# shionhonda/gae-dgl

Measured on AMD Instinct MI355X. Metric: edges aggregated/sec (SpMM fwd+bwd), higher is better.
Workload: dtype f32 (storage, aggregations, accumulators; the dense products run on the 16-bit matrix pipe from split operands with fp32 accumulation: X W^T and dW from three bf16 pieces per operand / six pairs, the loss from two fp16 pieces (N >= 5120) or three bf16 pieces -- all fp32-grade, see ms_per_step_exact_

## Files before the change

### gae_dgl_amd/csrc/common.h

```cpp
#pragma once
#include <hip/hip_runtime.h>
#include <stdint.h>
#include <stdio.h>

#include <atomic>

#include "gae_hip.h"
#include "gae_hip_experimental.h"

namespace gae {

struct Knob {
    std::atomic<int> v;
    explicit constexpr Knob(int x) : v(x) {}
    operator int() const { return v.load(std::memory_order_relaxed); }
    Knob &operator=(int x) { v.store(x, std::memory_order_relaxed); return *this; }
};

extern Knob g_spmm_variant, g_spmm_rpg, g_spmm_tile_vecs, g_spmm_ell, g_spmm_ell_rpg, g_spmm_hot, g_spmm_desc, g_spmm_light;
extern Knob g_gemm_rows, g_linear_wlds, g_atb_bf16, g_ell_side;
extern Knob g_xw_rows, g_xw_parts, g_xw_glds, g_xw_p3;
extern Knob g_bce_s_bf16, g_bce_pv_bf16, g_bce_sym, g_bce_sym_ri, g_bce_sym_bal, g_bce_last_kind;
extern Knob g_topk_splits;

// ... 119 lines not shown
struct PartialList {
    const float *base;
    float *out;
    int64_t n, n_partials, stride, row_len, row_pitch, out_pitch;
};
int launch_partials_reduce(const PartialList &a, const PartialList &b, hipStream_t s);

__device__ __forceinline__ void philox_round(uint32_t (&c)[4], uint32_t k0, uint32_t k1)
{
    const uint64_t p0 = uint64_t(0xD2511F53u) * c[0];
    const uint64_t p1 = uint64_t(0xCD9E8D57u) * c[2];
    const uint32_t n0 = uint32_t(p1 >> 32) ^ c[1] ^ k0;
    const uint32_t n2 = uint32_t(p0 >> 32) ^ c[3] ^ k1;
    c[1] = uint32_t(p1); c[3] = uint32_t(p0); c[0] = n0; c[2] = n2;
}

__device__ __forceinline__ void philox4x32_10(uint64_t ctr, uint64_t draw, uint64_t seed, uint32_t (&c)[4])
{
    c[0] = uint32_t(ctr); c[1] = uint32_t(ctr >> 32); c[2] = uint32_t(draw); c[3] = uint32_t(draw >> 32);
    uint32_t k0 = uint32_t(seed), k1 = uint32_t(seed >> 32);
#pragma unroll
    for (int r = 0; r < 10; ++r) {
        philox_round(c, k0, k1);
        k0 += 0x9E3779B9u; k1 += 0xBB67AE85u;
    }
}

__device__ __forceinline__ float dropout_multiplier(uint32_t bits, float p, float scale)
{
    const float u = float(bits >> 8) * (1.0f / 16777216.0f);
    return u >= p ? scale : 0.f;
}

}
```

### gae_dgl_amd/csrc/decoder_bce.hip

```cpp
#include <string.h>

#include "common.h"
#include "bce_finalize.h"

namespace {

using gae::kWave;
typedef float f32x4 __attribute__((ext_vector_type(4)));
typedef short s16x4 __attribute__((ext_vector_type(4)));
typedef float f32x2 __attribute__((ext_vector_type(2)));
typedef __bf16 bf16x2 __attribute__((ext_vector_type(2)));

constexpr int TJ = 64;
constexpr int PREP_ROWS = 64;
constexpr int kBceRi = 2;
constexpr int64_t kBceGrid = 2048;
constexpr int64_t kBceSymGrid = 16384;
constexpr int kChipCus = 256;
}

namespace gae {
Knob g_bce_s_bf16{3};
Knob g_bce_last_kind{0};
Knob g_bce_sym_bal{1};
// ... 25 lines not shown
#pragma unroll
    for (int r = 0; r < 4; ++r) {
        t[r] = 1.0f + __builtin_amdgcn_exp2f(-fabsf(y[r]));
        tA += fabsf(y[r]);
    }
    float t01, t23, q;
    if constexpr (SCALAR_TREE) {
        asm("v_mul_f32 %0, %1, %2" : "=v"(t01) : "v"(t[0]), "v"(t[1]));
        asm("v_mul_f32 %0, %1, %2" : "=v"(t23) : "v"(t[2]), "v"(t[3]));
        asm("v_mul_f32 %0, %1, %2" : "=v"(q) : "v"(t01), "v"(t23));
    } else {
        t01 = t[0] * t[1]; t23 = t[2] * t[3]; q = t01 * t23;
    }
    tP *= q;
    const float R = __builtin_amdgcn_rcpf(q);
    const float r01 = R * t23, r23 = R * t01;
    float s0, s1, s2, s3;
    asm("v_fma_f32 %0, %1, %2, -0.5" : "=v"(s0) : "v"(r01), "v"(t[1]));
    asm("v_fma_f32 %0, %1, %2, -0.5" : "=v"(s1) : "v"(r01), "v"(t[0]));
    asm("v_fma_f32 %0, %1, %2, -0.5" : "=v"(s2) : "v"(r23), "v"(t[3]));
    asm("v_fma_f32 %0, %1, %2, -0.5" : "=v"(s3) : "v"(r23), "v"(t[2]));
    return f32x4{copysignf(s0, y[0]), copysignf(s1, y[1]), copysignf(s2, y[2]), copysignf(s3, y[3])};
}

__global__ __launch_bounds__(256) void bce_prepare_kernel(const float *__restrict__ Z, float *__restrict__ mask,
                                                          int64_t ldz, int64_t n, int d, int DP, int64_t row_begin,
                                                          int64_t row_end, float *__restrict__ Zt,
                                                          unsigned short *__restrict__ Zhi,
                                                          unsigned short *__restrict__ Zlo,
                                                          double *__restrict__ colsum_partial ,
                                                          float drop_p, float drop_scale, uint64_t seed,
                                                          uint64_t offset, const uint64_t *__restrict__ draw_dev,
                                                          const int64_t *__restrict__ counts ,
                                                          double *__restrict__ scal , double all_pairs)
{
    __shared__ double red[2][256];
    const int tid = threadIdx.x;
    const int64_t n_valid = counts ? counts[0] : n;
    if (counts && blockIdx.x == 0 && tid == 0) {
        const double nv = double(counts[0]), ev = double(counts[1]);
        scal[0] = ev > 0 ? (nv * nv - ev) / ev : 0.0;
        scal[1] = nv > 0 ? 1.0 / (nv * nv) : 0.0;
        scal[2] = all_pairs - nv * nv;
    }
    const int k = tid % DP, rl = tid / DP, rpp = 256 / DP;
    const int64_t r0 = int64_t(blockIdx.x) * PREP_ROWS;
    double s_all = 0.0, s_win = 0.0;
    const bool draw = drop_p > 0.f;
    const uint64_t draw_idx = (draw && draw_dev) ? *draw_dev : 0;
    for (int rr = rl; rr < PREP_ROWS; rr += rpp) {
        const int64_t i = r0 + rr;
        if (i >= n) break;
        float v = 0.f;
        if (k < d && i >= n_valid) {
            if (draw) mask[i * ldz + k] = 0.f;
        } else if (k < d) {
            v = Z[i * ldz + k];
            if (draw) {
                const int64_t e = i * d + k;
                uint32_t c[4];
                gae::philox4x32_10(offset + uint64_t(e >> 2), draw_idx, seed, c);
                const uint32_t bits = (e & 2) ? ((e & 1) ? c[3] : c[2]) : ((e & 1) ? c[1] : c[0]);
                const float m = gae::dropout_multiplier(bits, drop_p, drop_scale);
                mask[i * ldz + k] = m;
                v *= m;
            } else if (mask) {
                v *= mask[i * ldz + k];
            }
        }
        Zt[i * DP + k] = v;
        const unsigned short hi = gae::f32_to_bf16(v);
        Zhi[i * DP + k] = hi;
        Zlo[i * DP + k] = gae::f32_to_bf16(v - gae::bf16_to_f32(hi));
        s_all += double(v);
        if (i >= row_begin && i < row_end) s_win += double(v);
    }
    red[0][tid] = s_all; red[1][tid] = s_win;
    __syncthreads();
    if (tid < DP) {
        double a = 0.0, w = 0.0;
        for (int q = 0; q < rpp; ++q) { a += red[0][q * DP + tid]; w += red[1][q * DP + tid]; }
        colsum_partial[(int64_t(blockIdx.x) * 2 + 0) * DP + tid] = a;
        colsum_partial[(int64_t(blockIdx.x) * 2 + 1) * DP + tid] = w;
    }
}

__device__ __forceinline__ void bce_colsum_block(const double *__restrict__ colsum_partial, int64_t n_blocks, int DP,
                                                 double *__restrict__ S ,
                                                 float *__restrict__ S_all_f , double *red )
{
    const int k = threadIdx.x % DP, q = threadIdx.x / DP, nq = 256 / DP;
    double a = 0.0, w = 0.0;
    for (int64_t b = q; b < n_blocks; b += nq) {
        a += colsum_partial[(b * 2 + 0) * DP + k];
        w += colsum_partial[(b * 2 + 1) * DP + k];
    }
    red[threadIdx.x] = a; red[256 + threadIdx.x] = w;
    __syncthreads();
    if (threadIdx.x < DP) {
        a = 0.0; w = 0.0;
        for (int j = 0; j < nq; ++j) { a += red[j * DP + k]; w += red[256 + j * DP + k]; }
        S[k] = a; S[DP + k] = w;
        S_all_f[k] = float(a);
    }
}

typedef short s16x8 __attribute__((ext_vector_type(8)));
typedef __bf16 bf16x8 __attribute__((ext_vector_type(8)));
// ... 41 lines not shown
    unsigned h[2], l[2], l2[2];
#pragma unroll
    for (int q = 0; q < 2; ++q) {
        const f32x2 a = {v[2 * q], v[2 * q + 1]};
        const unsigned hu = __builtin_bit_cast(unsigned, __builtin_convertvector(a, bf16x2));
        const f32x2 r1 = a - f32x2{__uint_as_float(hu << 16), __uint_as_float(hu & 0xffff0000u)};
        const unsigned lu = __builtin_bit_cast(unsigned, __builtin_convertvector(r1, bf16x2));
        const f32x2 r2 = r1 - f32x2{__uint_as_float(lu << 16), __uint_as_float(lu & 0xffff0000u)};
        h[q] = hu; l[q] = lu;
        l2[q] = __builtin_bit_cast(unsigned, __builtin_convertvector(r2, bf16x2));
    }
    struct U { unsigned a, b; } uh{h[0], h[1]}, ul{l[0], l[1]}, ul2{l2[0], l2[1]};
    hi = __builtin_bit_cast(s16x4, uh);
    lo = __builtin_bit_cast(s16x4, ul);
    lo2 = __builtin_bit_cast(s16x4, ul2);
}
__device__ __forceinline__ s16x4 third_piece(const f32x4 &v, const s16x4 &hi, const s16x4 &lo)
{
    unsigned l2[2];
#pragma unroll
    for (int q = 0; q < 2; ++q) {
        const f32x2 a = {v[2 * q], v[2 * q + 1]};
        const f32x2 fh = {gae::bf16_to_f32((unsigned short)hi[2 * q]), gae::bf16_to_f32((unsigned short)hi[2 * q + 1])};
        const f32x2 fl = {gae::bf16_to_f32((unsigned short)lo[2 * q]), gae::bf16_to_f32((unsigned short)lo[2 * q + 1])};
        l2[q] = __builtin_bit_cast(unsigned, __builtin_convertvector((a - fh) - fl, bf16x2));
    }
    struct U { unsigned a, b; } u{l2[0], l2[1]};
    return __builtin_bit_cast(s16x4, u);
}

typedef _Float16 f16x8 __attribute__((ext_vector_type(8)));
typedef _Float16 f16x4 __attribute__((ext_vector_type(4)));
typedef __fp16 fp16x2 __attribute__((ext_vector_type(2)));
constexpr float kF16Max = 32768.f;
__device__ __forceinline__ f32x4 mfma32h(const s16x8 &a, const s16x8 &b, const f32x4 &c)
{
    return __builtin_amdgcn_mfma_f32_16x16x32_f16(__builtin_bit_cast(f16x8, a), __builtin_bit_cast(f16x8, b), c, 0, 0, 0);
}
template <bool F16>
__device__ __forceinline__ f32x4 mfma_k32(const s16x8 &a, const s16x8 &b, const f32x4 &c)
{
    if constexpr (F16) return mfma32h(a, b, c);
    else return mfma32(a, b, c);
}
typedef _Float16 f16x2 __attribute__((ext_vector_type(2)));
__device__ __forceinline__ float minus_f16_lo(float v, unsigned hh)
{
    float r;
    asm("v_fma_mix_f32 %0, %1, -1.0, %2 op_sel_hi:[1,0,0]" : "=v"(r) : "v"(hh), "v"(v));
    return r;
}
__device__ __forceinline__ float minus_f16_hi(float v, unsigned hh)
{
    float r;
    asm("v_fma_mix_f32 %0, %1, -1.0, %2 op_sel:[1,0,0] op_sel_hi:[1,0,0]" : "=v"(r) : "v"(hh), "v"(v));
    return r;
}
__device__ __forceinline__ void split_f16x4(const f32x4 &v, s16x4 &hi, s16x4 &lo)
{
    unsigned h[2], l[2];
#pragma unroll
    for (int q = 0; q < 2; ++q) {
        const f32x2 a = {v[2 * q], v[2 * q + 1]};
        const unsigned hu = __builtin_bit_cast(unsigned, __builtin_convertvector(a, f16x2));
        const f32x2 r = {minus_f16_lo(a[0], hu), minus_f16_hi(a[1], hu)};
        h[q] = hu;
        l[q] = __builtin_bit_cast(unsigned, __builtin_convertvector(r, f16x2));
// ... 285 lines not shown
    }
#pragma unroll
    for (int off = 32; off > 0; off >>= 1) { la += __shfl_down(la, off, 64); ll += __shfl_down(ll, off, 64); }
    if (lane == 0) { red[wave][0] = la; red[wave][1] = ll; }
    __syncthreads();
    if (tid == 0) {
        const int64_t b = int64_t(blockIdx.y) * n_row_blocks + blockIdx.x;
        loss_partial[2 * b + 0] = (red[0][0] + red[1][0]) + (red[2][0] + red[3][0]);
        loss_partial[2 * b + 1] = (red[0][1] + red[1][1]) + (red[2][1] + red[3][1]);
    }
}

}

namespace gae {
Knob g_bce_sym_ri{0};
}

namespace {
using gae::g_bce_sym_ri;

__device__ __forceinline__ s16x4 upper_halves(const f32x4 &d)
{
    struct U { unsigned a, b; } u{__builtin_amdgcn_perm(__float_as_uint(d[1]), __float_as_uint(d[0]), 0x07060302u),
                                  __builtin_amdgcn_perm(__float_as_uint(d[3]), __float_as_uint(d[2]), 0x07060302u)};
    return __builtin_bit_cast(s16x4, u);
}

__host__ __device__ inline int64_t sym_strip_offset(int64_t I, int64_t NP, int64_t PR)
{
    return 16 * (I * NP - PR * (I * (I + 1) / 2));
}

template <bool WITH_GRAD, int RI, bool TRV, bool S3 = false, bool F16 = false, bool PERSIST = false, bool BAL = false>
__global__ __launch_bounds__(256, (RI == 2 && !PERSIST) ? 3 : 2) void bce_dense_sym_kernel(
    const float *__restrict__ Zt , const unsigned short *__restrict__ Zhi,
    const unsigned short *__restrict__ Zlo, int64_t n, int64_t cols_per_chunk,
    float *__restrict__ O_partial , float *__restrict__ Wmir,
    double *__restrict__ loss_partial , const double *__restrict__ colsum_partial,
    int64_t n_prep_blocks, double *__restrict__ S, float *__restrict__ S_all_f, unsigned n_panels, int exp_strip,
    unsigned *__restrict__ range_flag, int flag_mode, unsigned ticket, unsigned n_chunks, int bal_tpb)
{
    if (flag_mode == 2 && *range_flag != ticket) return;
    static_assert(!(S3 && F16), "three bf16 pieces OR two fp16 pieces");
    bool out_of_range = false;
    constexpr bool STAGE32 = S3 || F16;
    constexpr int DP = 16, SYM_PR = 64 * RI;
    constexpr int LDH = DP + 4;
    constexpr int V4 = TJ * DP / 4 / 256;
    constexpr int LDT = TJ + 4;
    constexpr int LDM = TJ + 4;
    constexpr int LDHL = 2 * DP + 8;
    __shared__ __attribute__((aligned(16))) unsigned short HLs[2][TJ * LDHL];
    __shared__ __attribute__((aligned(16))) unsigned short L2s[2][S3 ? TJ * LDH : 4];
    __shared__ __attribute__((aligned(16))) unsigned short HT[2][TRV ? 4 : DP * LDT];
    __shared__ __attribute__((aligned(16))) unsigned short LT[2][TRV ? 4 : DP * LDT];
    __shared__ __attribute__((aligned(16))) float MR[2][4][16 * LDM];
    __shared__ double red[4][2];

  double sumA = 0.0, sumL = 0.0;
  auto unit = [&](const int64_t I, const int64_t col_begin, const int64_t col_end, const int64_t op_slot, const int64_t lp_index) {
    const int tid = threadIdx.x, lane = tid & 63, wave = tid >> 6;
    const int l15 = lane & 15, g = lane >> 4;
    const int64_t NP = (n + 63) / 64 * 64;
    const int64_t row_base = SYM_PR * I + wave * (RI * 16);
    const int64_t diag_end = SYM_PR * (I + 1);

    constexpr float LOG2E = 1.44269504088896341f;
    static_assert(RI % 2 == 0, "row subtiles are paired into K = 32 mirror products");
    s16x8 bhh[RI];
    s16x8 bll[RI];
    s16x8 b3[S3 ? RI : 1];
    s16x8 zTh[RI / 2], zTl[RI / 2];
#pragma unroll
    for (int ri = 0; ri < RI; ++ri) {
        const int64_t i = row_base + ri * 16 + l15;
        f32x4 b = *reinterpret_cast<const f32x4 *>(Zt + (i < n ? i : 0) * DP + 4 * g);
        if (i >= n) b = f32x4{0.f, 0.f, 0.f, 0.f};
        b *= LOG2E;
        s16x4 bhi, blo, blo2;
        if (S3) { split_bf16x4_3(b, bhi, blo, blo2); b3[ri] = cat(bhi, blo2); }
        else if (F16) {
            out_of_range |= !(fmaxf(fmaxf(fabsf(b[0]), fabsf(b[1])), fmaxf(fabsf(b[2]), fabsf(b[3]))) <= kF16Max * LOG2E);
            split_f16x4(b, bhi, blo);
        } else split_bf16x4(b, bhi, blo);
        bhh[ri] = cat(bhi, bhi);
        bll[ri] = cat(blo, blo);
        s16x4 th, tl;
#pragma unroll
        for (int r = 0; r < 4; ++r) {
            const int64_t ir = row_base + ri * 16 + 4 * g + r;
            const bool v = ir < n;
            if (F16) continue;
            th[r] = v ? short(Zhi[(v ? ir : 0) * DP + l15]) : short(0);
            tl[r] = v ? short(Zlo[(v ? ir : 0) * DP + l15]) : short(0);
        }
        if (F16) {
            f32x4 zr;
#pragma unroll
            for (int r = 0; r < 4; ++r) {
                const int64_t ir = row_base + ri * 16 + 4 * g + r;
                zr[r] = ir < n ? Zt[ir * DP + l15] : 0.f;
            }
            split_f16x4(zr, th, tl);
        }
        put_half(zTh[ri / 2], ri & 1, th);
        put_half(zTl[ri / 2], ri & 1, tl);
    }
    s16x4 ident;
#pragma unroll
    for (int r = 0; r < 4; ++r) ident[r] = (4 * g + r == l15) ? short(F16 ? 0x3C00 : 0x3F80) : short(0);
    f32x4 oacc[RI];
#pragma unroll
    for (int ri = 0; ri < RI; ++ri) oacc[ri] = f32x4{0.f, 0.f, 0.f, 0.f};
    if (!BAL) { sumA = 0.0; sumL = 0.0; }
    bool rvalid[RI];
#pragma unroll
    for (int ri = 0; ri < RI; ++ri) rvalid[ri] = (row_base + ri * 16 + l15) < n;
// ... 5 lines not shown
#pragma unroll
            for (int r = 0; r < 4; ++r) pad_lane += (pad_j0 + jt * 16 + 4 * g + r >= n) ? 1.f : 0.f;
    }

    struct Stage { s16x4 h[STAGE32 ? 1 : V4], l[STAGE32 ? 1 : V4]; f32x4 f[STAGE32 ? V4 : 1]; };
    auto load_tile = [&](int64_t j0, Stage &st) {
#pragma unroll
        for (int q = 0; q < V4; ++q) {
            const int idx = tid + 256 * q;
            const int jj = idx / (DP / 4), kk = (idx % (DP / 4)) * 4;
            const bool jv = j0 + jj < col_end;
            const int64_t j = jv ? j0 + jj : col_begin;
            if (STAGE32) {
                st.f[q] = *reinterpret_cast<const f32x4 *>(Zt + j * DP + kk);
                if (!jv) st.f[q] = f32x4{0.f, 0.f, 0.f, 0.f};
            } else {
                st.h[q] = *reinterpret_cast<const s16x4 *>(Zhi + j * DP + kk);
                st.l[q] = *reinterpret_cast<const s16x4 *>(Zlo + j * DP + kk);
                if (!jv) { st.h[q] = s16x4{0, 0, 0, 0}; st.l[q] = s16x4{0, 0, 0, 0}; }
            }
        }
    };
    auto store_tile = [&](int buf, const Stage &st) {
#pragma unroll
        for (int q = 0; q < V4; ++q) {
            const int idx = tid + 256 * q;
            const int jj = idx / (DP / 4), kk = (idx % (DP / 4)) * 4;
            s16x4 h4, l4;
            if (S3) {
                s16x4 l24;
                split_bf16x4_3(st.f[q], h4, l4, l24);
                *reinterpret_cast<s16x4 *>(&L2s[buf][jj * LDH + kk]) = l24;
            } else if (F16) {
                const f32x4 f = st.f[q];
                out_of_range |= !(fmaxf(fmaxf(fabsf(f[0]), fabsf(f[1])), fmaxf(fabsf(f[2]), fabsf(f[3]))) <= kF16Max);
                split_f16x4(f, h4, l4);
            } else {
                h4 = st.h[q]; l4 = st.l[q];
            }
            *reinterpret_cast<s16x8 *>(&HLs[buf][jj * LDHL + 2 * kk]) = cat(h4, l4);
            if (WITH_GRAD && !TRV) {
#pragma unroll
                for (int e = 0; e < 4; ++e) {
                    HT[buf][(kk + e) * LDT + jj] = (unsigned short)h4[e];
                    LT[buf][(kk + e) * LDT + jj] = (unsigned short)l4[e];
                }
            }
        }
    };
    float *strip = Wmir + sym_strip_offset(I, NP, SYM_PR);
    auto flush_mirror = [&](int64_t j0, int mb) {
        const int f = tid >> 4, jq = (tid & 15) * 4;
        f32x4 v = *reinterpret_cast<const f32x4 *>(&MR[mb][0][f * LDM + jq]);
#pragma unroll
        for (int w = 1; w < 4; ++w) v += *reinterpret_cast<const f32x4 *>(&MR[mb][w][f * LDM + jq]);
        f32x4 *sp = reinterpret_cast<f32x4 *>(strip + (j0 - diag_end) * 16 + f * TJ + jq);
        if (exp_strip == 1) __builtin_nontemporal_store(v, sp);
        else if (exp_strip == 2) asm volatile("global_store_dwordx4 %0, %1, off sc1" ::"v"(sp), "v"(v) : "memory");
        else *sp = v;
    };

    auto compute_tile = [&](int buf, int64_t j0, bool offdiag) {
        float tA[RI], tP[RI];
#pragma unroll
        for (int ri = 0; ri < RI; ++ri) { tA[ri] = 0.f; tP[ri] = 1.f; }
#pragma unroll((RI == 4 && S3) ? 1 : TJ / 32)
        for (int jp = 0; jp < TJ / 32; ++jp) {
            s16x8 ph[RI], pl[RI];
#pragma unroll
// ... 81 lines not shown
#pragma unroll
        for (int ri = 0; ri < RI; ++ri) {
            a += rvalid[ri] ? tA[ri] : 0.f;
            l += rvalid[ri] ? __builtin_amdgcn_logf(tP[ri]) - padcnt : 0.f;
        }
        sumA += w * double(a);
        sumL += w * double(l);
    };

    Stage stage;
    load_tile(col_begin, stage);
    store_tile(0, stage);
    __syncthreads();
    int buf = 0;
    for (int64_t j0 = col_begin; j0 < col_end; j0 += TJ, buf ^= 1) {
        const bool more = j0 + TJ < col_end;
        if (more) load_tile(j0 + TJ, stage);
        const bool offdiag = j0 >= diag_end;
        compute_tile(buf, j0, offdiag);
        if (more) store_tile(buf ^ 1, stage);
        __syncthreads();
        if (WITH_GRAD && offdiag) flush_mirror(j0, buf);
    }
    if (WITH_GRAD) {
        float *op = O_partial + op_slot * n * DP;
#pragma unroll
        for (int ri = 0; ri < RI; ++ri)
#pragma unroll
            for (int r = 0; r < 4; ++r) {
                const int64_t i = row_base + ri * 16 + 4 * g + r;
                if (i < n) op[i * DP + l15] = oacc[ri][r];
            }
    }
    if (F16 && flag_mode == 1 && out_of_range) atomicExch(range_flag, ticket);
    if (BAL) return;
    double la = sumA * 0.69314718055994531, ll = sumL;
#pragma unroll
    for (int off = 32; off > 0; off >>= 1) { la += __shfl_down(la, off, 64); ll += __shfl_down(ll, off, 64); }
    if (lane == 0) { red[wave][0] = la; red[wave][1] = ll; }
    __syncthreads();
    if (tid == 0) {
        loss_partial[2 * lp_index + 0] = (red[0][0] + red[1][0]) + (red[2][0] + red[3][0]);
        loss_partial[2 * lp_index + 1] = (red[0][1] + red[1][1]) + (red[2][1] + red[3][1]);
    }
  };
  auto unit_xy = [&](const unsigned bx, const unsigned by) {
    if (bx >= n_panels) {
        if (by == 0)
            bce_colsum_block(colsum_partial, n_prep_blocks, DP, S, S_all_f, reinterpret_cast<double *>(&MR[0][0][0]));
        return;
    }
    const int64_t col_begin = SYM_PR * int64_t(bx) + int64_t(by) * cols_per_chunk;
    const int64_t lp_index = int64_t(by) * n_panels + bx;
    if (col_begin >= n) {
        if (threadIdx.x == 0) { loss_partial[2 * lp_index] = 0.0; loss_partial[2 * lp_index + 1] = 0.0; }
        return;
    }
    const int64_t ce = col_begin + cols_per_chunk;
    unit(bx, col_begin, ce > n ? n : ce, by, lp_index);
  };
    if constexpr (BAL) {
        const unsigned n_vb = n_chunks;
        auto vblock = [&](const unsigned vb) {
        if (vb + 1 == n_vb) {
            bce_colsum_block(colsum_partial, n_prep_blocks, DP, S, S_all_f, reinterpret_cast<double *>(&MR[0][0][0]));
            return;
        }
// ... 6 lines not shown
        if (t1 > W) t1 = W;
        if (t0 < t1) {
            const float hb = float(NT) + 0.5f * float(TPP);
            int I = int((hb - sqrtf(fmaxf(hb * hb - 2.0f * float(TPP) * float(t0), 0.0f))) / float(TPP));
            if (I < 0) I = 0;
            if (I > T - 1) I = T - 1;
            I = __builtin_amdgcn_readfirstlane(I);
            while (I > 0 && prefix(I) > t0) --I;
            while (I + 1 < T && prefix(I + 1) <= t0) ++I;
            while (t0 < t1) {
                const int pI = prefix(I), tiles = NT - TPP * I;
                const int lt = t0 - pI;
                int cnt = tiles - lt;
                if (cnt > t1 - t0) cnt = t1 - t0;
                const int64_t cb = int64_t(SYM_PR) * I + int64_t(lt) * 64;
                int64_t ce = cb + int64_t(cnt) * 64;
                if (ce > n) ce = n;
                if (cb < n) unit(I, cb, ce, int(vb) - int(unsigned(pI) / unsigned(bal_tpb)), -1);
                __syncthreads();
                t0 += cnt; ++I;
            }
        }
        const int tid = threadIdx.x, lane = tid & 63, wave = tid >> 6;
        double la = sumA * 0.69314718055994531, ll = sumL;
#pragma unroll
        for (int off = 32; off > 0; off >>= 1) { la += __shfl_down(la, off, 64); ll += __shfl_down(ll, off, 64); }
        if (lane == 0) { red[wave][0] = la; red[wave][1] = ll; }
        __syncthreads();
        if (tid == 0) {
            loss_partial[2 * vb + 0] = (red[0][0] + red[1][0]) + (red[2][0] + red[3][0]);
            loss_partial[2 * vb + 1] = (red[0][1] + red[1][1]) + (red[2][1] + red[3][1]);
        }
        };
        if constexpr (PERSIST) {
            for (unsigned vb = blockIdx.x; vb < n_vb; vb += gridDim.x) {
                vblock(vb);
                __syncthreads();
            }
        } else {
            vblock(blockIdx.x);
        }
    } else if constexpr (PERSIST) {
        const unsigned nx = n_panels + 1, total = nx * n_chunks;
        for (unsigned u = blockIdx.x; u < total; u += gridDim.x) {
            unit_xy(u % nx, u / nx);
            __syncthreads();
        }
    } else {
        unit_xy(blockIdx.x, blockIdx.y);
    }
}

__global__ __launch_bounds__(256) void bce_mirror_reduce_kernel(const float *__restrict__ Wmir, int64_t n,
                                                               float *__restrict__ Omir , int SYM_PR)
{
    const int64_t NP = (n + 63) / 64 * 64;
    const int64_t j0 = int64_t(blockIdx.x) * TJ;
    const int f = threadIdx.x >> 4, jq = (threadIdx.x & 15) * 4;
    const int64_t n_left = j0 / SYM_PR;
    f32x4 acc = {0.f, 0.f, 0.f, 0.f};
    auto at = [&](int64_t I) {
        const int64_t de = SYM_PR * (I + 1);
        return *reinterpret_cast<const f32x4 *>(Wmir + sym_strip_offset(I, NP, SYM_PR) + (j0 - de) * 16 + f * TJ + jq);
    };
    int64_t I = 0;
    for (; I + 8 <= n_left; I += 8) {
        f32x4 v[8];
#pragma unroll
        for (int u = 0; u < 8; ++u) v[u] = at(I + u);
#pragma unroll
        for (int u = 0; u < 8; ++u) acc += v[u];
    }
    for (; I < n_left; ++I) acc += at(I);
#pragma unroll
    for (int e = 0; e < 4; ++e)
        if (j0 + jq + e < n) Omir[(j0 + jq + e) * 16 + f] = acc[e];
}

template <int VEC, int LPR, bool WITH_GRAD>
__global__ __launch_bounds__(256) void bce_edges_kernel(
    const float *__restrict__ Zt , const float *__restrict__ mask, int64_t ldz,
    int64_t row_begin, int64_t n_local, int d, const int32_t *__restrict__ indptr,
    const int32_t *__restrict__ indices, const int32_t *__restrict__ t_indptr, const int32_t *__restrict__ t_indices,
// ... 454 lines not shown
    GAE_REQUIRE((Z || prepared) && loss_out && workspace && (n_local == 0 || indptr), GAE_E_NULL, "gae_decoder_bce: NULL pointer");
    GAE_REQUIRE(!dZ || n_local == 0 || t_indptr, GAE_E_NULL, "gae_decoder_bce: the gradient needs the CSR of A^T");
    BcePlan p;
    bce_plan(n, n_local, d, true, p);
    GAE_REQUIRE(workspace_bytes >= p.total_bytes, GAE_E_WORKSPACE, "gae_decoder_bce: workspace %lld < %lld bytes",
                (long long)workspace_bytes, (long long)p.total_bytes);
    if (prepared) {
        GAE_REQUIRE(prepared_blocks >= 1 && prepared_blocks * 2 * p.DP * 8 <= p.cs_bytes, GAE_E_RANGE,
                    "gae_x_decoder_bce_prepared: %lld column-sum partials do not fit the workspace", (long long)prepared_blocks);
        p.prep_blocks = prepared_blocks;
    }
    GAE_REQUIRE(gae::aligned16(workspace), GAE_E_ALIGN, "gae_decoder_bce: workspace not 16-byte aligned");
    hipStream_t s = gae::as_stream(stream);
    char *w = static_cast<char *>(workspace);
    float *O = reinterpret_cast<float *>(w); w += p.o_bytes;
    float *Zt = reinterpret_cast<float *>(w); w += p.zt_bytes;
    unsigned short *Zhi = reinterpret_cast<unsigned short *>(w); w += p.zh_bytes;
    unsigned short *Zlo = reinterpret_cast<unsigned short *>(w); w += p.zh_bytes;
    double *cs = reinterpret_cast<double *>(w); w += p.cs_bytes;
    double *S = reinterpret_cast<double *>(w);
    float *S_all_f = reinterpret_cast<float *>(w + 2 * p.DP * 8);
    double *scal = counts ? reinterpret_cast<double *>(w + 2 * p.DP * 8 + ((p.DP * 4 + 7) & ~7)) : nullptr;
    unsigned *range_flag = reinterpret_cast<unsigned *>(w + 2 * p.DP * 8 + ((p.DP * 4 + 7) & ~7) + 3 * 8);
    w += p.s_bytes;
    double *lp = reinterpret_cast<double *>(w); w += align256((2 * p.n_dense + p.edge_blocks) * 8);
    float *Wmir = reinterpret_cast<float *>(w); w += p.wmir_bytes;
    float *Omir = reinterpret_cast<float *>(w);
    const double inv_n2 = 1.0 / (double(n) * double(n));
    if (n_local == 0) {
        GAE_HIP(hipMemsetAsync(loss_out, 0, sizeof(float), s));
        if (t_tail_out) { memset(t_tail_out, 0, sizeof(gae_bce_tail)); t_tail_out = nullptr; }
        return GAE_OK;
    }
    if (!prepared) {
        hipLaunchKernelGGL(bce_prepare_kernel, dim3(unsigned(p.prep_blocks)), dim3(256), 0, s, Z, mask, ldz, n, int(d), p.DP,
                           row_begin, row_begin + n_local, Zt, Zhi, Zlo, cs, dropout_p, 1.0f / (1.0f - dropout_p), seed,
                           offset, draw_dev, counts, scal, bce_all_pairs(p, n, n_local));
        GAE_CHECK_LAUNCH("bce_prepare_kernel");
    }
    int rc;
    g_bce_last_kind = p.sym ? (p.sym_pr == 256 ? 3 : 2) : 1;
    if (p.sym) {
        const dim3 grid = p.bal_tpb ? dim3(unsigned(p.bal_blocks) + 1) : dim3(unsigned(p.row_blocks) + 1, unsigned(p.n_splits));
        static std::atomic<unsigned> call_counter{0};
        const unsigned ticket = (call_counter.fetch_add(1) * 2654435761u) | 0x80000001u;
#define GAE_SYM3(WG, R, T, S3V, F16V, FM, PERS, GRID)                                                                \
    do { if (p.bal_tpb) GAE_SYM4(WG, R, T, S3V, F16V, FM, PERS, true, GRID); else GAE_SYM4(WG, R, T, S3V, F16V, FM, PERS, false, GRID); } while (0)
#define GAE_SYM4(WG, R, T, S3V, F16V, FM, PERS, BALV, GRID)                                                          \
    hipLaunchKernelGGL((bce_dense_sym_kernel<WG, R, T, S3V, F16V, PERS, BALV>), GRID, dim3(256), 0, s, Zt, Zhi, Zlo, n, p.cols_per_split, O, Wmir, \
                       lp, cs, p.prep_blocks, S, S_all_f, unsigned(p.row_blocks),                                    \
                       n >= 32768 ? 1 : 0, range_flag, FM, ticket,                                                   \
                       (p.bal_tpb ? unsigned(p.bal_blocks) + 1u : unsigned(p.n_splits)), p.bal_tpb)
#define GAE_SYM(WG, R, T) do { if (g_bce_s_bf16 == 3) { GAE_SYM3(WG, R, T, false, true, 1, false, grid); GAE_SYM3(WG, R, T, true, false, 2, true, (p.bal_tpb ? dim3(64) : dim3(2 * kChipCus))); } \
    else GAE_SYM3(WG, R, T, true, false, 0, false, grid); } while (0)
        if (!dZ) { if (p.sym_pr == 256) GAE_SYM(false, 4, false); else GAE_SYM(false, 2, false); }
        else { if (p.sym_pr == 256) GAE_SYM(true, 4, true); else GAE_SYM(true, 2, true); }
#undef GAE_SYM
#undef GAE_SYM3
#undef GAE_SYM4
        GAE_CHECK_LAUNCH("bce_dense_sym_kernel");
        if (dZ && p.LPR != 4) {
            hipLaunchKernelGGL(bce_mirror_reduce_kernel, dim3(unsigned((n + TJ - 1) / TJ)), dim3(256), 0, s, Wmir, n,
                               Omir, p.sym_pr);
            GAE_CHECK_LAUNCH("bce_mirror_reduce_kernel");
        }
        rc = GAE_OK;
    } else {
        rc = dZ ? launch_dense<true>(p, Zt, Zhi, Zlo, n, row_begin, n_local, O, lp, cs, S, S_all_f, s)
                : launch_dense<false>(p, Zt, Zhi, Zlo, n, row_begin, n_local, O, lp, cs, S, S_all_f, s);
    }
    if (rc) return rc;
    double *lpe = lp + 2 * p.n_dense;
    rc = dZ ? launch_edges<4, true>(p, Zt, mask, ldz, row_begin, n_local, int(d), indptr, indices, t_indptr, t_indices,
                                    pos_weight, float(inv_n2), O, S_all_f, dZ, lddz, lpe, p.sym ? Omir : nullptr,
                                    counts, scal, (p.sym && p.LPR == 4) ? Wmir : nullptr,
                                    p.sym ? range_flag : nullptr, s)
            : launch_edges<4, false>(p, Zt, mask, ldz, row_begin, n_local, int(d), indptr, indices, t_indptr,
                                     t_indices, pos_weight, float(inv_n2), O, S_all_f, dZ, lddz, lpe, nullptr, counts,
                                     scal, nullptr, p.sym ? range_flag : nullptr, s);
    if (rc) return rc;
    gae_bce_tail tail;
    memset(&tail, 0, sizeof(tail));
    tail.dense_partial = lp; tail.n_dense = p.n_dense;
    tail.edge_partial = lpe; tail.n_edge = p.edge_blocks;
    tail.S = S; tail.DP = p.DP;
    tail.pad_terms = p.pad_terms; tail.inv_n2 = inv_n2;
    tail.loss_out = loss_out; tail.bump_draw = dropout_p > 0.f ? draw_dev : nullptr; tail.scal = scal;
// ... 97 lines not shown
```

### gae_dgl_amd/csrc/spmm_ell.hip

```cpp
#include <string.h>

#include <utility>

#include "common.h"

namespace {

typedef unsigned u32x4 __attribute__((ext_vector_type(4)));
typedef float f32x4 __attribute__((ext_vector_type(4)));

constexpr int32_t kEllOverflow = -2;
constexpr int32_t kEllSkip = -3;

template <int CTRL, int BANK>
__device__ __forceinline__ unsigned dpp_mov(unsigned old, unsigned v)
{
    return unsigned(__builtin_amdgcn_update_dpp(int(old), int(v), CTRL, 0xF, BANK, false));
}

template <int LP16, int K>
__device__ __forceinline__ unsigned bcast_slot(unsigned v)
{
    constexpr int ROW_NEWBCAST = 0x150;
    if constexpr (LP16 == 16) {
// ... 82 lines not shown
    const void *H;
    void *M;
    const float *row_scale, *col_scale;
    int64_t n_rows, ldm;
    unsigned ldh_bytes, h_bytes;
    unsigned n_cols, F, nvec;
    unsigned n_row_blocks, n_ftiles, tile_vecs;
    int xcd_tiled, store_pad, store_mode;
    const float *W, *bias;
    float *Y;
    int64_t ldy;
    int J, w_so, w_sk, act, store_m;
    const float *ep_bias;
    int ep_act;
    const void *Hmask;
    int n_splits;
    unsigned split_bytes, empty_off;
    const float *W2, *bias2;
    int w_split, w_t;
    const float *sw_P, *sw_Q;
    float *sw_part;
    int64_t sw_ldp, sw_ldq, sw_stride;
    int sw_O, sw_I, sw_variant;
    float *pz_t;
    unsigned short *pz_hi, *pz_lo;
    double *pz_cs, *pz_scal;
    float *pz_mask;
    int64_t pz_ldmask;
    float pz_drop_p, pz_drop_scale;
    uint64_t pz_seed, pz_offset;
    const uint64_t *pz_draw;
    const int64_t *pz_counts;
    double pz_all_pairs;
};

template <typename T>
__device__ __forceinline__ void store16(T *p, const u32x4 w, int mode)
{
    if (mode == 2) {
        asm volatile("global_store_dwordx4 %0, %1, off sc1\n\ts_nop 1" ::"v"(p), "v"(w) : "memory");
    } else if (mode == 1) {
        __builtin_nontemporal_store(w, reinterpret_cast<u32x4 *>(p));
    } else {
        *reinterpret_cast<u32x4 *>(p) = w;
    }
}
__device__ __forceinline__ void store_elem(float *p, float v) { *p = v; }
__device__ __forceinline__ void store_elem(unsigned short *p, float v) { *p = gae::f32_to_bf16(v); }

template <int LP16, int B0, int NREG, int... U>
__device__ __forceinline__ void slot_offsets(const unsigned (&off)[NREG], unsigned add, unsigned (&out)[sizeof...(U)],
                                             std::integer_sequence<int, U...>)
{
    ((out[U] = bcast_slot<LP16, (B0 + U) % LP16>(off[(B0 + U) / LP16]) + add), ...);
}

__device__ __forceinline__ u32x4 relu_gate(u32x4 v, const u32x4 m)
{
#pragma unroll
    for (int i = 0; i < 4; ++i) v[i] = __uint_as_float(m[i]) > 0.f ? v[i] : 0u;
    return v;
}

template <typename T, int LP16, int RPG, int NREG, int B0, int N, bool SCALED, int MODE>
__device__ __forceinline__ void ell_slots(__amdgpu_buffer_rsrc_t rs_h, __amdgpu_buffer_rsrc_t rs_c,
                                          __amdgpu_buffer_rsrc_t rs_m,
// ... 183 lines not shown
    static_assert(W % NB == 0 && NB % 4 == 0, "slots are consumed in whole batches");
    unsigned blk, ftile;
    if (a.xcd_tiled) {
        const unsigned xcd = blockIdx.x % gae::kNumXcd, k = blockIdx.x / gae::kNumXcd;
        const unsigned tl = k / a.n_row_blocks;
        blk = k - tl * a.n_row_blocks;
        ftile = xcd + gae::kNumXcd * tl;
        if (ftile >= a.n_ftiles) return;
    } else {
        blk = gae::xcd_remap(blockIdx.x, gridDim.x);
        ftile = blockIdx.y;
    }
    const int lane = threadIdx.x & 63;
    const int lig = threadIdx.x % LPR, grp = threadIdx.x / LPR;
    const unsigned fvec = ftile * a.tile_vecs + lig;
    const bool live = unsigned(lig) < a.tile_vecs && fvec < a.nvec;
    const unsigned lane_off = fvec * 16u;

    constexpr int SW_ROWS = 256 / LPR;
    constexpr int SWP = EPI_J > 0 ? SW_ROWS * 32 / 256 : 1, SWQ = EPI_J > 0 ? SW_ROWS * 64 / 256 : 1;
    __shared__ float SwP[EPI_J > 0 ? SW_ROWS * 32 : 1], SwQ[EPI_J > 0 ? SW_ROWS * 64 : 1];
    float swp[SWP], swq[SWQ];
    constexpr int JPL_K = EPI_J > 0 ? EPI_J / LPR : 1;
    int64_t pz_n_valid = a.n_rows;
    uint64_t pz_draw_idx = 0;
    if constexpr (EPI_J == 16) {
        if (a.pz_t != nullptr) {
            if (a.pz_counts) pz_n_valid = a.pz_counts[0];
            if (a.pz_drop_p > 0.f && a.pz_draw) pz_draw_idx = *a.pz_draw;
        }
    }
    double pz_sum[JPL_K];
    float pz_m[JPL_K];
#pragma unroll
    for (int q = 0; q < JPL_K; ++q) pz_m[q] = 1.f;
#pragma unroll
    for (int q = 0; q < JPL_K; ++q) pz_sum[q] = 0.0;
    constexpr int SW_K = EPI_J > 0 ? SW_ROWS / 4 : 1;
    float sda[SW_K], sdb[SW_K];
    bool sw_direct = false;
    int sd_mt = 0, sd_nt = 0;
    bool sd_ones = false, sd_live = false;
    if constexpr (EPI_J > 0) {
        if (a.sw_part != nullptr && (a.sw_variant & 8)) {
            const int mt_n = (a.sw_O + 15) >> 4, nt_n = (a.sw_I + 15) >> 4;
            sw_direct = mt_n * nt_n + mt_n <= 4;
            if (sw_direct) {
                const int tile = 3 - int(threadIdx.x >> 6);
                sd_live = tile < mt_n * nt_n + mt_n;
                sd_ones = tile < mt_n;
                const int pt = tile - mt_n;
                sd_mt = sd_ones ? tile : pt / nt_n;
                sd_nt = sd_ones ? 0 : pt - sd_mt * nt_n;
                const int l15 = threadIdx.x & 15, g4 = (threadIdx.x & 63) >> 4;
                const int o = sd_mt * 16 + l15, i = sd_nt * 16 + l15;
#pragma unroll
                for (int st = 0; st < SW_K; ++st) {
                    const int64_t rw = int64_t(blk) * SW_ROWS + 4 * st + g4;
                    const bool okr = sd_live && rw < a.n_rows;
                    const bool oka = okr && o < a.sw_O, okb = okr && !sd_ones && i < a.sw_I;
                    const float av = a.sw_P[oka ? rw * a.sw_ldp + o : 0];
                    const float bv = a.sw_Q[okb ? rw * a.sw_ldq + i : 0];
                    sda[st] = oka ? av : 0.f;
                    sdb[st] = sd_ones ? 1.f : (okb ? bv : 0.f);
                }
            }
// ... 166 lines not shown
        }
        if constexpr (EPI_J > 0) {
            constexpr int JPL = EPI_J / LPR;
            float yv[JPL];
#pragma unroll
            for (int q = 0; q < JPL; ++q) yv[q] = 0.f;
#pragma unroll
            for (int j = 0; j < EPI_J; ++j) {
                const f32x4 w = *reinterpret_cast<const f32x4 *>(&Ws[j * LDW + 4 * lig]);
                float p = fmaf(acc[r][3], w[3], fmaf(acc[r][2], w[2], fmaf(acc[r][1], w[1], acc[r][0] * w[0])));
                p = group_allreduce<LPR>(p);
                if (j / JPL == lig) yv[j % JPL] = p;
            }
            if (row[r] < a.n_rows) {
#pragma unroll
                for (int q = 0; q < JPL; ++q) {
                    const int o = lig * JPL + q;
                    if (o < a.J) {
                        float y = yv[q] + (a.bias ? ((a.bias2 != nullptr && o >= a.w_split) ? a.bias2[o - a.w_split] : a.bias[o]) : 0.f);
                        if (a.act == GAE_ACT_RELU) y = fmaxf(y, 0.f);
                        a.Y[row[r] * a.ldy + o] = y;
                        yv[q] = y;
                    }
                }
            }
            if constexpr (EPI_J == 16) {
                if (a.pz_t != nullptr) {
                    const bool in = row[r] < a.n_rows;
#pragma unroll
                    for (int q = 0; q < JPL; ++q) {
                        const int o = lig * JPL + q;
                        const float v = (in && o < a.J) ? yv[q] * pz_m[q] : 0.f;
                        if (in) {
                            a.pz_t[row[r] * 16 + o] = v;
                            const unsigned short hi = gae::f32_to_bf16(v);
                            a.pz_hi[row[r] * 16 + o] = hi;
                            a.pz_lo[row[r] * 16 + o] = gae::f32_to_bf16(v - gae::bf16_to_f32(hi));
                        }
                        pz_sum[q] = double(v);
                    }
                }
            }
        }
    }
    if constexpr (EPI_J == 16) {
        if (a.pz_t != nullptr) {
            double *cred = reinterpret_cast<double *>(SwQ);
#pragma unroll
            for (int q = 0; q < JPL_K; ++q) {
#pragma unroll
                for (int off = LPR; off < 64; off <<= 1) pz_sum[q] += __shfl_xor(pz_sum[q], off, 64);
                if ((threadIdx.x & 63) < LPR) cred[(threadIdx.x >> 6) * 16 + lig * JPL_K + q] = pz_sum[q];
            }
            __syncthreads();
            if (threadIdx.x < 16) {
                const double t = ((cred[threadIdx.x] + cred[16 + threadIdx.x]) + cred[32 + threadIdx.x]) + cred[48 + threadIdx.x];
                a.pz_cs[(int64_t(blk) * 2 + 0) * 16 + threadIdx.x] = t;
                a.pz_cs[(int64_t(blk) * 2 + 1) * 16 + threadIdx.x] = t;
            }
            if (a.pz_counts && blk == 0 && threadIdx.x == 0) {
                const double nv = double(a.pz_counts[0]), ev = double(a.pz_counts[1]);
                a.pz_scal[0] = ev > 0 ? (nv * nv - ev) / ev : 0.0;
                a.pz_scal[1] = nv > 0 ? 1.0 / (nv * nv) : 0.0;
                a.pz_scal[2] = a.pz_all_pairs - nv * nv;
            }
        }
    }
    if constexpr (EPI_J > 0) {
        if (a.sw_part != nullptr && sw_direct) {
            if (sd_live) {
                const int O = a.sw_O, I = a.sw_I;
                const int l15 = threadIdx.x & 15, g4 = (threadIdx.x & 63) >> 4;
                typedef float f32x4_t __attribute__((ext_vector_type(4)));
                f32x4_t acc = {0.f, 0.f, 0.f, 0.f};
#pragma unroll
                for (int st = 0; st < SW_K; ++st) acc = __builtin_amdgcn_mfma_f32_16x16x4f32(sda[st], sdb[st], acc, 0, 0, 0);
                float *pp = a.sw_part + int64_t(blk) * a.sw_stride;
                const int i = sd_nt * 16 + l15;
#pragma unroll
                for (int q = 0; q < 4; ++q) {
                    const int oo = sd_mt * 16 + 4 * g4 + q;
                    if (sd_ones) { if (oo < O && l15 == 0) pp[O * I + oo] = acc[q]; }
                    else if (oo < O && i < I) pp[oo * I + i] = acc[q];
                }
            }
        } else if (a.sw_part != nullptr) {
            const int O = a.sw_O, I = a.sw_I;
#pragma unroll
            for (int q = 0; q < SWP; ++q) SwP[threadIdx.x + 256 * q] = swp[q];
#pragma unroll
            for (int q = 0; q < SWQ; ++q) SwQ[threadIdx.x + 256 * q] = swq[q];
            __syncthreads();
            float *pp = a.sw_part + int64_t(blk) * a.sw_stride;
            if (a.sw_variant & 4) {
                const int wv = threadIdx.x >> 6, l15 = threadIdx.x & 15, g4 = (threadIdx.x & 63) >> 4;
                const int mt_n = (O + 15) >> 4, nt_n = (I + 15) >> 4;
                for (int tile = 3 - wv; tile < mt_n * nt_n + mt_n; tile += 4) {
                    const bool ones = tile < mt_n;
// ... 191 lines not shown
    if (n_rows == 0) return GAE_OK;
    GAE_REQUIRE(indptr && H && W && Y, GAE_E_NULL, "gae_gcn_layer_fused: NULL pointer");
    GAE_REQUIRE(ldh >= F && ldh % 4 == 0 && gae::aligned16(H), GAE_E_ALIGN,
                "gae_gcn_layer_fused: rows of H must be whole 16-byte vectors");
    GAE_REQUIRE(!M || (ldm >= F && ldm % 4 == 0 && gae::aligned16(M)), GAE_E_ALIGN,
                "gae_gcn_layer_fused: rows of M must be whole 16-byte vectors");
    GAE_REQUIRE(ldy >= J, GAE_E_SIZE, "gae_gcn_layer_fused: ldy < J");
    GAE_REQUIRE(n_cols > 0 && n_cols * ldh * 4 + (int64_t(1) << 16) < (int64_t(1) << 32), GAE_E_SIZE,
                "gae_gcn_layer_fused: H larger than a raw buffer resource addresses");
    EllArgs a{};
    a.indptr = indptr; a.indices = indices; a.ell = plan->ell;
    a.H = H; a.M = M; a.row_scale = row_scale; a.col_scale = col_scale;
    a.n_rows = n_rows; a.ldm = M ? ldm : 0;
    a.ldh_bytes = unsigned(ldh * 4);
    a.h_bytes = unsigned(n_cols * ldh * 4);
    a.empty_off = a.h_bytes; a.n_splits = 1;
    a.n_cols = unsigned(n_cols); a.F = unsigned(F); a.nvec = unsigned((F + 3) / 4);
    a.tile_vecs = a.nvec;
    a.xcd_tiled = 0; a.store_pad = 0; a.store_mode = 0;
    a.W = W; a.bias = bias; a.Y = Y; a.ldy = ldy; a.J = int(J); a.w_so = int(w_stride_out); a.w_sk = int(w_stride_in);
    a.act = act; a.store_m = M != nullptr;
    a.W2 = W2; a.bias2 = bias2; a.w_split = int(w_split); a.w_t = w_transposed;
    if (side) {
        a.sw_P = side->P; a.sw_Q = side->Q; a.sw_part = side->part;
        a.sw_ldp = side->ldp; a.sw_ldq = side->ldq; a.sw_stride = side->stride; a.sw_O = side->O; a.sw_I = side->I;
        a.sw_variant = int(gae::g_ell_side);
    }
    if (prep) {
        a.pz_t = prep->lay->Zt; a.pz_hi = prep->lay->Zhi; a.pz_lo = prep->lay->Zlo; a.pz_cs = prep->lay->colsum_partial;
        a.pz_scal = prep->lay->scal; a.pz_all_pairs = prep->lay->all_pairs;
        a.pz_mask = prep->mask; a.pz_ldmask = prep->ldmask; a.pz_drop_p = prep->drop_p;
        a.pz_drop_scale = 1.0f / (1.0f - prep->drop_p);
        a.pz_seed = prep->seed; a.pz_offset = prep->offset; a.pz_draw = prep->draw; a.pz_counts = prep->counts;
    }
    hipStream_t s = gae::as_stream(stream);
    const bool scaled = row_scale != nullptr;
    const int ew = plan->ell_width;
    if (a.nvec <= 8) return J <= 16 ? launch_ell_epi_w<8, 16>(a, ew, scaled, s) : launch_ell_epi_w<8, 32>(a, ew, scaled, s);
    return J <= 16 ? launch_ell_epi_w<16, 16>(a, ew, scaled, s) : launch_ell_epi_w<16, 32>(a, ew, scaled, s);
}

extern "C" int gae_x_gcn_layer_fused_prep(const int32_t *indptr, const int32_t *indices, int64_t n, const float *H,
                                        int64_t ldh, float *M, int64_t ldm, int64_t F, const float *row_scale,
                                        const float *col_scale, const gae_spmm_plan *plan, const float *W,
                                        int64_t w_stride_out, int64_t w_stride_in, const float *bias, int64_t J,
                                        float *Z, int64_t ldz, const gae_bce_prep *prep, float *mask, int64_t ldmask,
                                        float dropout_p, uint64_t seed, uint64_t offset, const uint64_t *draw_dev,
                                        const int64_t *counts_dev, int64_t *n_prep_blocks_out, void *stream)
{
    GAE_REQUIRE(prep && n_prep_blocks_out, GAE_E_NULL, "gae_x_gcn_layer_fused_prep: NULL pointer");
    GAE_REQUIRE(J >= 1 && J <= 16 && prep->DP == 16, GAE_E_RANGE,
                "gae_x_gcn_layer_fused_prep: the embedding must be at most 16 wide (got %lld)", (long long)J);
    GAE_REQUIRE(dropout_p >= 0.f && dropout_p < 1.f, GAE_E_RANGE, "gae_x_gcn_layer_fused_prep: dropout_p outside [0, 1)");
    GAE_REQUIRE(dropout_p == 0.f || mask, GAE_E_NULL, "gae_x_gcn_layer_fused_prep: dropout_p > 0 needs the mask output buffer");
    GAE_REQUIRE(!mask || ldmask >= J, GAE_E_SIZE, "gae_x_gcn_layer_fused_prep: ldmask < J");
    GAE_REQUIRE(n >= 1, GAE_E_SIZE, "gae_x_gcn_layer_fused_prep: empty graph");
    const int64_t rpb = (F + 3) / 4 <= 8 ? 32 : 16, blocks = (n + rpb - 1) / rpb;
    GAE_REQUIRE(blocks <= prep->max_blocks && prep->Zt && prep->Zhi && prep->Zlo && prep->colsum_partial, GAE_E_WORKSPACE,
                "gae_x_gcn_layer_fused_prep: layout not from gae_x_decoder_bce_prep_layout for this n");
    *n_prep_blocks_out = blocks;
    FusedPrep fp{prep, mask, ldmask, dropout_p, seed, offset, draw_dev, counts_dev};
    return gcn_layer_fused_impl(indptr, indices, n, n, H, ldh, M, ldm, F, row_scale, col_scale, plan, W, w_stride_out,
                                w_stride_in, bias, J, GAE_ACT_IDENTITY, Z, ldz, nullptr, nullptr, 0, 0, stream, nullptr, &fp);
}

static int64_t fused_wgrad_blocks(int64_t n_rows, int64_t F) { const int64_t rpb = (F + 3) / 4 <= 8 ? 32 : 16; return (n_rows + rpb - 1) / rpb; }
// ... 132 lines not shown
```

Measured before the change: 1.313 billion.

## Move fp16 range check into prepare stage and drop the fallback relaunch

The fp16-split range check moves out of the dense symmetric BCE kernel and into the prepare kernels (standalone and fused into the ELL GCN epilogue), which write a ticket flag. The dense kernel now reads the flag at entry and picks the three-bf16 body or the fp16 body inside one launch. This removes the second persistent fallback launch that always ran and early-exited, and it drops the per-element range checks from the hot loop. The risk is that the fused path writes its flag into scal+3, which assumes spare space there, and that the flag must be in place before the dense kernel reads it.

```diff
diff --git a/gae_dgl_amd/csrc/common.h b/gae_dgl_amd/csrc/common.h
--- a/gae_dgl_amd/csrc/common.h
+++ b/gae_dgl_amd/csrc/common.h
@@ -175,4 +175,12 @@
     return u >= p ? scale : 0.f;
 }
 
+constexpr float kF16Max = 32768.f;
+__device__ __forceinline__ bool f16_pieces_out_of_range(float v) { return !(fabsf(v) <= kF16Max); }
+inline unsigned next_range_ticket()
+{
+    static std::atomic<unsigned> counter{0};
+    return (counter.fetch_add(1) * 2654435761u) | 0x80000001u;
 }
+
+}
diff --git a/gae_dgl_amd/csrc/decoder_bce.hip b/gae_dgl_amd/csrc/decoder_bce.hip
--- a/gae_dgl_amd/csrc/decoder_bce.hip
+++ b/gae_dgl_amd/csrc/decoder_bce.hip
@@ -81,9 +81,12 @@
                                                           float drop_p, float drop_scale, uint64_t seed,
                                                           uint64_t offset, const uint64_t *__restrict__ draw_dev,
                                                           const int64_t *__restrict__ counts ,
-                                                          double *__restrict__ scal , double all_pairs)
+                                                          double *__restrict__ scal , double all_pairs,
+                                                          unsigned *__restrict__ range_flag ,
+                                                          unsigned ticket)
 {
     __shared__ double red[2][256];
+    bool out_of_range = false;
     const int tid = threadIdx.x;
     const int64_t n_valid = counts ? counts[0] : n;
     if (counts && blockIdx.x == 0 && tid == 0) {
@@ -118,11 +121,16 @@
             }
         }
         Zt[i * DP + k] = v;
+        out_of_range |= gae::f16_pieces_out_of_range(v);
         const unsigned short hi = gae::f32_to_bf16(v);
         Zhi[i * DP + k] = hi;
         Zlo[i * DP + k] = gae::f32_to_bf16(v - gae::bf16_to_f32(hi));
         s_all += double(v);
         if (i >= row_begin && i < row_end) s_win += double(v);
+    }
+    if (range_flag != nullptr) {
+        if (blockIdx.x == 0 && tid == 0) range_flag[1] = ticket;
+        if (out_of_range) range_flag[0] = ticket;
     }
     red[0][tid] = s_all; red[1][tid] = s_win;
     __syncthreads();
@@ -230,7 +238,6 @@
 typedef _Float16 f16x8 __attribute__((ext_vector_type(8)));
 typedef _Float16 f16x4 __attribute__((ext_vector_type(4)));
 typedef __fp16 fp16x2 __attribute__((ext_vector_type(2)));
-constexpr float kF16Max = 32768.f;
 __device__ __forceinline__ f32x4 mfma32h(const s16x8 &a, const s16x8 &b, const f32x4 &c)
 {
     return __builtin_amdgcn_mfma_f32_16x16x32_f16(__builtin_bit_cast(f16x8, a), __builtin_bit_cast(f16x8, b), c, 0, 0, 0);
@@ -582,18 +589,27 @@
     return 16 * (I * NP - PR * (I * (I + 1) / 2));
 }
 
-template <bool WITH_GRAD, int RI, bool TRV, bool S3 = false, bool F16 = false, bool PERSIST = false, bool BAL = false>
-__global__ __launch_bounds__(256, (RI == 2 && !PERSIST) ? 3 : 2) void bce_dense_sym_kernel(
-    const float *__restrict__ Zt , const unsigned short *__restrict__ Zhi,
+template <bool S3, bool TRV>
+struct SymLds {
+    static constexpr int DP = 16, LDH = DP + 4, LDT = TJ + 4, LDM = TJ + 4, LDHL = 2 * DP + 8;
+    __attribute__((aligned(16))) unsigned short HLs[2][TJ * LDHL];
+    __attribute__((aligned(16))) unsigned short L2s[2][S3 ? TJ * LDH : 4];
+    __attribute__((aligned(16))) unsigned short HT[2][TRV ? 4 : DP * LDT];
+    __attribute__((aligned(16))) unsigned short LT[2][TRV ? 4 : DP * LDT];
+    __attribute__((aligned(16))) float MR[2][4][16 * LDM];
+    double red[4][2];
+};
+
+template <bool WITH_GRAD, int RI, bool TRV, bool S3, bool F16, bool BAL, class Lds>
+__device__ __forceinline__ void bce_dense_sym_body(
+    Lds &lds, const float *__restrict__ Zt , const unsigned short *__restrict__ Zhi,
     const unsigned short *__restrict__ Zlo, int64_t n, int64_t cols_per_chunk,
     float *__restrict__ O_partial , float *__restrict__ Wmir,
     double *__restrict__ loss_partial , const double *__restrict__ colsum_partial,
     int64_t n_prep_blocks, double *__restrict__ S, float *__restrict__ S_all_f, unsigned n_panels, int exp_strip,
-    unsigned *__restrict__ range_flag, int flag_mode, unsigned ticket, unsigned n_chunks, int bal_tpb)
-{
-    if (flag_mode == 2 && *range_flag != ticket) return;
+    unsigned n_chunks, int bal_tpb)
+{
     static_assert(!(S3 && F16), "three bf16 pieces OR two fp16 pieces");
-    bool out_of_range = false;
     constexpr bool STAGE32 = S3 || F16;
     constexpr int DP = 16, SYM_PR = 64 * RI;
     constexpr int LDH = DP + 4;
@@ -601,12 +617,12 @@
     constexpr int LDT = TJ + 4;
     constexpr int LDM = TJ + 4;
     constexpr int LDHL = 2 * DP + 8;
-    __shared__ __attribute__((aligned(16))) unsigned short HLs[2][TJ * LDHL];
-    __shared__ __attribute__((aligned(16))) unsigned short L2s[2][S3 ? TJ * LDH : 4];
-    __shared__ __attribute__((aligned(16))) unsigned short HT[2][TRV ? 4 : DP * LDT];
-    __shared__ __attribute__((aligned(16))) unsigned short LT[2][TRV ? 4 : DP * LDT];
-    __shared__ __attribute__((aligned(16))) float MR[2][4][16 * LDM];
-    __shared__ double red[4][2];
+    auto &HLs = lds.HLs;
+    auto &L2s = lds.L2s;
+    auto &HT = lds.HT;
+    auto &LT = lds.LT;
+    auto &MR = lds.MR;
+    auto &red = lds.red;
 
   double sumA = 0.0, sumL = 0.0;
   auto unit = [&](const int64_t I, const int64_t col_begin, const int64_t col_end, const int64_t op_slot, const int64_t lp_index) {
@@ -630,10 +646,8 @@
         b *= LOG2E;
         s16x4 bhi, blo, blo2;
         if (S3) { split_bf16x4_3(b, bhi, blo, blo2); b3[ri] = cat(bhi, blo2); }
-        else if (F16) {
-            out_of_range |= !(fmaxf(fmaxf(fabsf(b[0]), fabsf(b[1])), fmaxf(fabsf(b[2]), fabsf(b[3]))) <= kF16Max * LOG2E);
-            split_f16x4(b, bhi, blo);
-        } else split_bf16x4(b, bhi, blo);
+        else if (F16) split_f16x4(b, bhi, blo);
+        else split_bf16x4(b, bhi, blo);
         bhh[ri] = cat(bhi, bhi);
         bll[ri] = cat(blo, blo);
         s16x4 th, tl;
@@ -705,9 +719,7 @@
                 split_bf16x4_3(st.f[q], h4, l4, l24);
                 *reinterpret_cast<s16x4 *>(&L2s[buf][jj * LDH + kk]) = l24;
             } else if (F16) {
-                const f32x4 f = st.f[q];
-                out_of_range |= !(fmaxf(fmaxf(fabsf(f[0]), fabsf(f[1])), fmaxf(fabsf(f[2]), fabsf(f[3]))) <= kF16Max);
-                split_f16x4(f, h4, l4);
+                split_f16x4(st.f[q], h4, l4);
             } else {
                 h4 = st.h[q]; l4 = st.l[q];
             }
@@ -855,7 +867,6 @@
                 if (i < n) op[i * DP + l15] = oacc[ri][r];
             }
     }
-    if (F16 && flag_mode == 1 && out_of_range) atomicExch(range_flag, ticket);
     if (BAL) return;
     double la = sumA * 0.69314718055994531, ll = sumL;
 #pragma unroll
@@ -928,23 +939,31 @@
             loss_partial[2 * vb + 1] = (red[0][1] + red[1][1]) + (red[2][1] + red[3][1]);
         }
         };
-        if constexpr (PERSIST) {
-            for (unsigned vb = blockIdx.x; vb < n_vb; vb += gridDim.x) {
-                vblock(vb);
-                __syncthreads();
-            }
-        } else {
-            vblock(blockIdx.x);
-        }
-    } else if constexpr (PERSIST) {
-        const unsigned nx = n_panels + 1, total = nx * n_chunks;
-        for (unsigned u = blockIdx.x; u < total; u += gridDim.x) {
-            unit_xy(u % nx, u / nx);
-            __syncthreads();
-        }
+        vblock(blockIdx.x);
     } else {
         unit_xy(blockIdx.x, blockIdx.y);
     }
+}
+
+template <bool WITH_GRAD, int RI, bool TRV, bool S3 = false, bool F16 = false, bool BAL = false>
+__global__ __launch_bounds__(256, RI == 2 ? 3 : 2) void bce_dense_sym_kernel(
+    const float *__restrict__ Zt , const unsigned short *__restrict__ Zhi,
+    const unsigned short *__restrict__ Zlo, int64_t n, int64_t cols_per_chunk,
+    float *__restrict__ O_partial , float *__restrict__ Wmir,
+    double *__restrict__ loss_partial , const double *__restrict__ colsum_partial,
+    int64_t n_prep_blocks, double *__restrict__ S, float *__restrict__ S_all_f, unsigned n_panels, int exp_strip,
+    const unsigned *__restrict__ range_flag, unsigned n_chunks, int bal_tpb)
+{
+    __shared__ SymLds<S3 || F16, TRV> lds;
+    if constexpr (F16) {
+        if (range_flag[0] == range_flag[1]) {
+            bce_dense_sym_body<WITH_GRAD, RI, TRV, true, false, BAL>(lds, Zt, Zhi, Zlo, n, cols_per_chunk, O_partial, Wmir,
+                loss_partial, colsum_partial, n_prep_blocks, S, S_all_f, n_panels, exp_strip, n_chunks, bal_tpb);
+            return;
+        }
+    }
+    bce_dense_sym_body<WITH_GRAD, RI, TRV, S3, F16, BAL>(lds, Zt, Zhi, Zlo, n, cols_per_chunk, O_partial, Wmir,
+        loss_partial, colsum_partial, n_prep_blocks, S, S_all_f, n_panels, exp_strip, n_chunks, bal_tpb);
 }
 
 __global__ __launch_bounds__(256) void bce_mirror_reduce_kernel(const float *__restrict__ Wmir, int64_t n,
@@ -1465,27 +1484,25 @@
         if (t_tail_out) { memset(t_tail_out, 0, sizeof(gae_bce_tail)); t_tail_out = nullptr; }
         return GAE_OK;
     }
+    const bool f16 = p.sym && g_bce_s_bf16 == 3;
     if (!prepared) {
         hipLaunchKernelGGL(bce_prepare_kernel, dim3(unsigned(p.prep_blocks)), dim3(256), 0, s, Z, mask, ldz, n, int(d), p.DP,
                            row_begin, row_begin + n_local, Zt, Zhi, Zlo, cs, dropout_p, 1.0f / (1.0f - dropout_p), seed,
-                           offset, draw_dev, counts, scal, bce_all_pairs(p, n, n_local));
+                           offset, draw_dev, counts, scal, bce_all_pairs(p, n, n_local), f16 ? range_flag : nullptr,
+                           gae::next_range_ticket());
         GAE_CHECK_LAUNCH("bce_prepare_kernel");
     }
     int rc;
     g_bce_last_kind = p.sym ? (p.sym_pr == 256 ? 3 : 2) : 1;
     if (p.sym) {
         const dim3 grid = p.bal_tpb ? dim3(unsigned(p.bal_blocks) + 1) : dim3(unsigned(p.row_blocks) + 1, unsigned(p.n_splits));
-        static std::atomic<unsigned> call_counter{0};
-        const unsigned ticket = (call_counter.fetch_add(1) * 2654435761u) | 0x80000001u;
-#define GAE_SYM3(WG, R, T, S3V, F16V, FM, PERS, GRID)                                                                \
-    do { if (p.bal_tpb) GAE_SYM4(WG, R, T, S3V, F16V, FM, PERS, true, GRID); else GAE_SYM4(WG, R, T, S3V, F16V, FM, PERS, false, GRID); } while (0)
-#define GAE_SYM4(WG, R, T, S3V, F16V, FM, PERS, BALV, GRID)                                                          \
-    hipLaunchKernelGGL((bce_dense_sym_kernel<WG, R, T, S3V, F16V, PERS, BALV>), GRID, dim3(256), 0, s, Zt, Zhi, Zlo, n, p.cols_per_split, O, Wmir, \
-                       lp, cs, p.prep_blocks, S, S_all_f, unsigned(p.row_blocks),                                    \
-                       n >= 32768 ? 1 : 0, range_flag, FM, ticket,                                                   \
-                       (p.bal_tpb ? unsigned(p.bal_blocks) + 1u : unsigned(p.n_splits)), p.bal_tpb)
-#define GAE_SYM(WG, R, T) do { if (g_bce_s_bf16 == 3) { GAE_SYM3(WG, R, T, false, true, 1, false, grid); GAE_SYM3(WG, R, T, true, false, 2, true, (p.bal_tpb ? dim3(64) : dim3(2 * kChipCus))); } \
-    else GAE_SYM3(WG, R, T, true, false, 0, false, grid); } while (0)
+#define GAE_SYM3(WG, R, T, S3V, F16V)                                                                                \
+    do { if (p.bal_tpb) GAE_SYM4(WG, R, T, S3V, F16V, true); else GAE_SYM4(WG, R, T, S3V, F16V, false); } while (0)
+#define GAE_SYM4(WG, R, T, S3V, F16V, BALV)                                                                          \
+    hipLaunchKernelGGL((bce_dense_sym_kernel<WG, R, T, S3V, F16V, BALV>), grid, dim3(256), 0, s, Zt, Zhi, Zlo, n, p.cols_per_split, \
+                       O, Wmir, lp, cs, p.prep_blocks, S, S_all_f, unsigned(p.row_blocks), n >= 32768 ? 1 : 0,    \
+                       range_flag, (p.bal_tpb ? unsigned(p.bal_blocks) + 1u : unsigned(p.n_splits)), p.bal_tpb)
+#define GAE_SYM(WG, R, T) do { if (f16) GAE_SYM3(WG, R, T, false, true); else GAE_SYM3(WG, R, T, true, false); } while (0)
         if (!dZ) { if (p.sym_pr == 256) GAE_SYM(false, 4, false); else GAE_SYM(false, 2, false); }
         else { if (p.sym_pr == 256) GAE_SYM(true, 4, true); else GAE_SYM(true, 2, true); }
 #undef GAE_SYM
diff --git a/gae_dgl_amd/csrc/spmm_ell.hip b/gae_dgl_amd/csrc/spmm_ell.hip
--- a/gae_dgl_amd/csrc/spmm_ell.hip
+++ b/gae_dgl_amd/csrc/spmm_ell.hip
@@ -138,6 +138,8 @@
     const uint64_t *pz_draw;
     const int64_t *pz_counts;
     double pz_all_pairs;
+    unsigned *pz_range;
+    unsigned pz_ticket;
 };
 
 template <typename T>
@@ -387,6 +389,7 @@
     }
     double pz_sum[JPL_K];
     float pz_m[JPL_K];
+    bool pz_oor = false;
 #pragma unroll
     for (int q = 0; q < JPL_K; ++q) pz_m[q] = 1.f;
 #pragma unroll
@@ -619,6 +622,7 @@
                         const int o = lig * JPL + q;
                         const float v = (in && o < a.J) ? yv[q] * pz_m[q] : 0.f;
                         if (in) {
+                            pz_oor |= gae::f16_pieces_out_of_range(v);
                             a.pz_t[row[r] * 16 + o] = v;
                             const unsigned short hi = gae::f32_to_bf16(v);
                             a.pz_hi[row[r] * 16 + o] = hi;
@@ -651,6 +655,8 @@
                 a.pz_scal[1] = nv > 0 ? 1.0 / (nv * nv) : 0.0;
                 a.pz_scal[2] = a.pz_all_pairs - nv * nv;
             }
+            if (blk == 0 && threadIdx.x == 0) a.pz_range[1] = a.pz_ticket;
+            if (pz_oor) a.pz_range[0] = a.pz_ticket;
         }
     }
     if constexpr (EPI_J > 0) {
@@ -908,6 +914,8 @@
         a.pz_mask = prep->mask; a.pz_ldmask = prep->ldmask; a.pz_drop_p = prep->drop_p;
         a.pz_drop_scale = 1.0f / (1.0f - prep->drop_p);
         a.pz_seed = prep->seed; a.pz_offset = prep->offset; a.pz_draw = prep->draw; a.pz_counts = prep->counts;
+        a.pz_range = reinterpret_cast<unsigned *>(prep->lay->scal + 3);
+        a.pz_ticket = gae::next_range_ticket();
     }
     hipStream_t s = gae::as_stream(stream);
     const bool scaled = row_scale != nullptr;
```

Result: no change. 1.319 billion, median of 6 (+0.5%).
